# zhaozijie2022/LocoTouch

Hardware: AMD Instinct MI355X
Metric: env-steps/sec (whole node), TransportTeacher 4096 envs/GPU (higher is better)
Workload: dtype f32

## Files before the change

### locotouch_amd/_abi.py

```python
from __future__ import annotations

import ctypes
import os
import re

_HERE = os.path.dirname(os.path.abspath(__file__))
REPO = os.path.dirname(_HERE)
LIB_PATH = os.environ.get("LOCOTOUCH_AMD_LIB", os.path.join(_HERE, "_lib", "liblocotouch_env.so"))

_SCALARS = {"int": ctypes.c_int, "int32_t": ctypes.c_int32, "int64_t": ctypes.c_int64, "uint8_t": ctypes.c_uint8,
            "uint32_t": ctypes.c_uint32, "uint64_t": ctypes.c_uint64, "size_t": ctypes.c_size_t, "float": ctypes.c_float,
            "double": ctypes.c_double}
_DECL = re.compile(r"(?:const\s+)?(\w+)\s*((?:\*\s*(?:const\b\s*)?)*)(\w*)\s*((?:\[[^\]]*\]\s*)*)")


def _ctype(decl, structs, opaque, consts, typed, param):
    m = _DECL.fullmatch(decl.strip())
    if not m:
        return None
    base, stars, name, dims = m.groups()
    depth = stars.count("*")
    try:
        dims = [sum(int(t) if t.strip().isdigit() else consts[t.strip()] for t in d.split("+")) for d in re.findall(r"\[([^\]]*)\]", dims)]
    except KeyError:
# ... 62 lines not shown
        for attr in ("extra_reward_terms", "extra_termination_terms", "extra_observation_terms", "reward_term_params"):
            if hasattr(self, attr):
                v = getattr(self, attr)
                setattr(new, attr, dict(v) if isinstance(v, dict) else list(v))
        return new

    def to_dict(self) -> dict:
        def py(v):
            return [py(x) for x in v] if hasattr(v, "__len__") else v

        return {name: py(getattr(self, name)) for name, *_ in self._fields_ if not name.startswith("_")}


_ENV_VALUE_QUERIES = (
    "lt_abi_version", "lt_cfg_sizeof", "lt_cfg_num_presets", "lt_cfg_preset_id", "lt_cfg_obs_dim", "lt_cfg_tactile_dim", "lt_last_error",
    "lt_wgrad_splits", "lt_wgrad_ws_floats", "lt_elu_backward_bias_ws_floats", "lt_head_wgrad_ws_floats", "lt_adam_clip_step_ws_floats",
    "lt_elu_backward_bias_nblk", "lt_head_wgrad_nblk", "lt_mlp_backward_blocks", "lt_env_kernel_name", "lt_mlp_kernel_name")

HEADERS = (
    ("", "lt_env.h", False, _ENV_VALUE_QUERIES, ("lt_cfg", "lt_view", "lt_mlp_desc", "lt_render_view", "lt_render_desc")),
    ("OBS_NORM", "lt_obs_norm.h", False, (), ()),
    ("STUDENT", "lt_student.h", True, ("lt_student_step_launches",), ("lt_student_desc", "lt_student_params")),
    ("COLLECT", "lt_collect.h", False, (), ()),
    ("LEDGER", "lt_ledger.h", False, (), ()),
    ("CNN_TRAIN", "lt_cnn_train.h", False, ("lt_cnn_launches",), ("lt_cnn_desc", "lt_cnn_params", "lt_cnn_grads")),
    ("BC", "lt_bc.h", False, (), ()),
    ("LSTM", "lt_lstm.h", False, (), ()),
    ("MEMORY", "lt_memory.h", False, (), ("lt_memory_net",)),
    ("MEMORY_SEQ", "lt_memory_seq.h", False, ("lt_memory_seq_backward_units",), ("lt_memory_seq_net", "lt_memory_seq_grad")),
    ("MEMORY_GRU", "lt_memory_gru.h", False, ("lt_memory_gru_seq_backward_units",),
     ("lt_memory_gru_net", "lt_memory_gru_seq_net", "lt_memory_gru_seq_grad")),
    ("POLICY", "lt_policy.h", True, ("lt_policy_step_launches",), ("lt_policy_desc", "lt_policy_memory")),
    ("PPO_OPTS", "lt_ppo_opts.h", False, (), ()),
    ("MLP_DX", "lt_mlp_dx.h", True, (), ()),
    ("PPO_SYM", "lt_ppo_sym.h", False, (), ()),
    ("ENCODER", "lt_encoder.h", False, ("lt_encoder_forward_launches",), ("lt_encoder_desc", "lt_encoder_net")),
)


def _bind(table, include_dir):
    bound, seen, env_structs = [], set(), None
    for prefix, fname, uses_env_structs, queries, _ in table:
        path, queries = os.path.join(include_dir, fname), frozenset(queries)
        consts, structs, sigs = parse_header(open(path).read(), structs=env_structs if uses_env_structs else None, bases={"lt_cfg": _CfgMethods})
        if not prefix:
            env_structs = structs
        for name in sorted(queries - set(sigs)):
            raise ImportError(f"include/{fname}: the value query {name} named in _abi.HEADERS is not declared there")
        for name, (restype, _) in sigs.items():
            if name in seen:
                raise ImportError(f"include/{fname}: {name} repeats an entry point of an earlier header")
            if restype is not ctypes.c_int and (prefix or name not in queries):
                raise ImportError(f"include/{fname}: {name} returns no int (a new value query of lt_env.h belongs in _abi.HEADERS)")
        seen.update(sigs)
        bound.append((path, consts, structs, sigs, queries))
    return bound


ALL_SIGNATURES: dict = {}
ALL_VALUE_QUERIES: set = set()
for (_prefix, _, _, _, _published), (_path, _consts, _structs, _sigs, _queries) in zip(HEADERS, _bind(HEADERS, os.path.join(REPO, "include"))):
    _p = _prefix + "_" if _prefix else ""
    globals().update(_consts)
    globals().update({_p + "HEADER": _path, _p + "CONSTS": _consts, _p + "SIGNATURES": _sigs, _p + "VALUE_QUERIES": _queries})
    globals().update({_structs[_c].__name__: _structs[_c] for _c in _published})
    if not _prefix:
# ... 100 lines not shown
```

### locotouch_amd/csrc/lt_ppo.hip

```cpp
#include <hip/hip_runtime.h>
#include <math.h>
#include <stdint.h>

#include "lt_env.h"
#include "lt_host_check.h"
#include "lt_internal.h"
#include "lt_ppo_device.h"

namespace {

template <bool LOG, bool NORM>
__global__ __launch_bounds__(256) void lt_ppo_loss_kernel(const float* __restrict__ mu, const float* __restrict__ stdp, const float* __restrict__ value,
                                                          const float* __restrict__ actions, const float* __restrict__ old_logp,
                                                          const float* __restrict__ adv, const float* __restrict__ returns,
                                                          const float* __restrict__ old_values, const float* __restrict__ old_mu,
                                                          const float* __restrict__ old_sigma, const long long* __restrict__ idx,
                                                          long long M, int A, float clip, float vcoef, int clipped_value,
                                                          const float* __restrict__ adv_stats, float* __restrict__ dmu, float* __restrict__ dvalue, float* __restrict__ acc) {
  const long long row = (long long)blockIdx.x * 256 + threadIdx.x;
  const bool ok = row < M;
  const long long src = (ok && idx) ? idx[row] : row;
  __shared__ float sigma_lds[MAX_A];
  if constexpr (LOG) {
    if ((int)threadIdx.x < A) sigma_lds[threadIdx.x] = lt_sigma_of_log(stdp[threadIdx.x]);
    __syncthreads();
  }
  float part[4 + MAX_A];
  float amax_mu = 0.f, amax_v = 0.f;
#pragma unroll
  for (int i = 0; i < 4 + MAX_A; ++i) part[i] = 0.f;
  if (ok) {
    const float inv_m = 1.f / (float)M;
    float logp = 0.f, kl = 0.f;
    float z[MAX_A], isg[MAX_A];
#pragma unroll
    for (int a = 0; a < MAX_A; ++a) {
      if (a < A) {
        const float sg = LOG ? sigma_lds[a] : stdp[a], m = mu[row * A + a], x = actions[src * A + a];
        const float om = old_mu[src * A + a], os = old_sigma[src * A + a];
        isg[a] = 1.f / sg;
        z[a] = (x - m) * isg[a];
        logp += lt_ppo_logp_term<LOG>(z[a], sg, stdp[a]);
        kl += lt_ppo_kl_term(sg, os, om, m);
      }
    }
    float advr = adv[src];
    if constexpr (NORM) advr = (advr - adv_stats[0]) * adv_stats[1];
    const float ratio = __expf(logp - old_logp[src]);
    LT_PPO_SURROGATE(advr, ratio, clip, s1, s2, dsurr_dratio)
    const float dlogp = dsurr_dratio * ratio * inv_m;
#pragma unroll
    for (int a = 0; a < MAX_A; ++a) {
      if (a < A) {
        dmu[row * A + a] = dlogp * z[a] * isg[a];
        amax_mu = fmaxf(amax_mu, fabsf(dlogp * z[a] * isg[a]));
        if constexpr (LOG) part[4 + a] = dlogp * (z[a] * z[a] - 1.f);
        else part[4 + a] = dlogp * (z[a] * z[a] - 1.f) * isg[a];
      }
    }
    const float v = value[row], R = returns[src];
    float vl, dv;
    LT_PPO_VALUE_LOSS(v, R, old_values, src, clip, clipped_value, vl, dv)
    dvalue[row] = vcoef * dv * inv_m;
    amax_v = fabsf(vcoef * dv * inv_m);
    part[0] = fmaxf(s1, s2);
    part[1] = vl;
    part[2] = kl;
  }
  LT_PPO_BLOCK_REDUCE(part, amax_mu, amax_v, A, acc, false)
}

__global__ __launch_bounds__(64) void lt_ppo_finalize_kernel(const float* __restrict__ acc, const float* __restrict__ stdp, int A, float inv_m,
                                                             float vcoef, float ecoef, int std_is_log, float* __restrict__ out) {
  lt_ppo_finalize(acc, stdp, A, inv_m, vcoef, ecoef, std_is_log, out);
}

constexpr int EB_ROWS = 48;

__global__ __launch_bounds__(256) void lt_elu_bwd_bias_kernel(const float* da, const float* __restrict__ a, long long M, int N, float alpha,
                                                              float* dz, float* __restrict__ ws, float* __restrict__ amax) {
  const int n4 = N >> 2, lanes = 256 / n4;
  const int c4 = threadIdx.x % n4, rl = threadIdx.x / n4;
  const long long r0 = (long long)blockIdx.x * EB_ROWS;
  float4 sum = {0.f, 0.f, 0.f, 0.f};
  float mx = 0.f;
  if (rl < lanes) {
    for (int r = rl; r < EB_ROWS; r += lanes) {
      const long long row = r0 + r;
      if (row >= M) break;
      const float4 g = ((const float4*)(da + row * N))[c4], y = ((const float4*)(a + row * N))[c4];
      float4 o;
// ... 72 lines not shown
        s[u].x += v.x; s[u].y += v.y; s[u].z += v.z; s[u].w += v.w;
        b += RL;
      }
    }
  }
  __shared__ float4 red[256];
  red[threadIdx.x] = make_float4((s[0].x + s[1].x) + (s[2].x + s[3].x), (s[0].y + s[1].y) + (s[2].y + s[3].y),
                                 (s[0].z + s[1].z) + (s[2].z + s[3].z), (s[0].w + s[1].w) + (s[2].w + s[3].w));
  __syncthreads();
  if (lane == 0 && e < count) {
    float4 t = red[c];
    for (int l = 1; l < RL; ++l) { const float4 v = red[l * cols + c]; t.x += v.x; t.y += v.y; t.z += v.z; t.w += v.w; }
    const float o[4] = {t.x, t.y, t.z, t.w};
#pragma unroll
    for (int i = 0; i < 4; ++i) {
      const int ei = e + i;
      if (ei >= count) break;
      if (ei < split) J.out0[j][ei] = o[i];
      else if (J.out1[j]) J.out1[j][ei - split] = o[i];
    }
  }
}

void launch_one_sum(const float* ws, int nblk, long long stride, int count, int split, float* out0, float* out1, hipStream_t stream) {
  SumJobs J = {};
  J.njobs = 1;
  J.ws[0] = ws; J.out0[0] = out0; J.out1[0] = out1; J.stride[0] = stride;
  J.nblk[0] = nblk; J.count[0] = count; J.split[0] = split;
  const int epb = 256 / sum_row_lanes(nblk) * 4;
  J.first[1] = (count + epb - 1) / epb;
  hipLaunchKernelGGL(lt_partial_sums_kernel, dim3((unsigned)J.first[1]), dim3(256), 0, stream, J);
}

constexpr int HW_ROWS = 96, HW_MAX_N = 16;

template <int NN>
__global__ __launch_bounds__(256) void lt_head_wgrad_kernel(const float* __restrict__ dy, const float* __restrict__ x, int x_split, long long M, int n, int k,
                                                            float* __restrict__ ws) {
  const int k4 = k >> 2, lanes = 256 / k4;
  const int c4 = threadIdx.x % k4, rl = threadIdx.x / k4;
  const long long r0 = (long long)blockIdx.x * HW_ROWS;
  float4 acc[NN];
  float accb[NN];
#pragma unroll
  for (int j = 0; j < NN; ++j) { acc[j] = {0.f, 0.f, 0.f, 0.f}; accb[j] = 0.f; }
  if (rl < lanes) {
    for (int r = rl; r < HW_ROWS; r += 4 * lanes) {
      float4 xv[4];
      float d[4][NN];
#pragma unroll
      for (int u = 0; u < 4; ++u) {
        const long long row = r0 + r + u * lanes;
        const bool ok = (r + u * lanes) < HW_ROWS && row < M;
        xv[u] = ok ? ((const float4*)(x + row * k))[c4] : float4{0.f, 0.f, 0.f, 0.f};
        if (x_split) {
          const unsigned w[4] = {__float_as_uint(xv[u].x), __float_as_uint(xv[u].y), __float_as_uint(xv[u].z), __float_as_uint(xv[u].w)};
          float f[4];
#pragma unroll
          for (int i = 0; i < 4; ++i)
            f[i] = (float)__builtin_bit_cast(_Float16, (unsigned short)(w[i] & 0xFFFFu)) + (float)__builtin_bit_cast(_Float16, (unsigned short)(w[i] >> 16)) * (1.f / 64.f);
          xv[u] = float4{f[0], f[1], f[2], f[3]};
        }
#pragma unroll
        for (int j = 0; j < NN; ++j) d[u][j] = (ok && j < n) ? dy[row * n + j] : 0.f;
      }
#pragma unroll
      for (int u = 0; u < 4; ++u)
#pragma unroll
        for (int j = 0; j < NN; ++j) {
          acc[j].x += d[u][j] * xv[u].x; acc[j].y += d[u][j] * xv[u].y; acc[j].z += d[u][j] * xv[u].z; acc[j].w += d[u][j] * xv[u].w;
          accb[j] += d[u][j];
        }
    }
  }
  extern __shared__ float4 red[];
  float* const redb = (float*)(red + (size_t)lanes * NN * k4);
  if (rl < lanes) {
#pragma unroll
    for (int j = 0; j < NN; ++j) red[((size_t)rl * NN + j) * k4 + c4] = acc[j];
    if (c4 == 0)
#pragma unroll
      for (int j = 0; j < NN; ++j) redb[rl * NN + j] = accb[j];
  }
  __syncthreads();
  float* const out = ws + (size_t)blockIdx.x * ((size_t)n * k + HW_MAX_N);
  for (int e = threadIdx.x; e < n * k4; e += 256) {
    const int j = e / k4, c = e - j * k4;
    float4 t = red[(size_t)j * k4 + c];
    for (int l = 1; l < lanes; ++l) {
      const float4 u = red[((size_t)l * NN + j) * k4 + c];
      t.x += u.x; t.y += u.y; t.z += u.z; t.w += u.w;
    }
    ((float4*)(out + (size_t)j * k))[c] = t;
  }
  if (threadIdx.x < n) {
    float t = redb[threadIdx.x];
    for (int l = 1; l < lanes; ++l) t += redb[l * NN + threadIdx.x];
    out[(size_t)n * k + threadIdx.x] = t;
  }
}

__global__ __launch_bounds__(256) void lt_gae_kernel(const float* __restrict__ rewards, const unsigned char* __restrict__ dones,
                                                     const float* __restrict__ values, const float* __restrict__ last_values, float gamma,
                                                     float lam, int T, long long N, float* __restrict__ returns, float* __restrict__ advantages) {
  const long long e = (long long)blockIdx.x * 256 + threadIdx.x;
  if (e >= N) return;
  float next_v = last_values[e], gae = 0.f;
  for (int t = T - 1; t >= 0; --t) {
    const long long o = (long long)t * N + e;
    const float v = values[o], alive = 1.f - (float)dones[o];
    const float delta = rewards[o] + alive * gamma * next_v - v;
    gae = delta + alive * gamma * lam * gae;
    const float ret = gae + v;
    returns[o] = ret;
    advantages[o] = ret - v;
    next_v = v;
  }
}

constexpr int AD_PER_BLOCK = 2048;

__global__ __launch_bounds__(256) void lt_sumsq_kernel(const float* __restrict__ g, long long n, float* __restrict__ ws) {
  const long long base = (long long)blockIdx.x * AD_PER_BLOCK;
  float s = 0.f;
  for (int k = threadIdx.x; k < AD_PER_BLOCK; k += 256) {
    const long long i = base + k;
    if (i < n) s += g[i] * g[i];
  }
  for (int off = 32; off > 0; off >>= 1) s += __shfl_xor(s, off, 64);
  __shared__ float red[4];
  if ((threadIdx.x & 63) == 0) red[threadIdx.x >> 6] = s;
  __syncthreads();
  if (threadIdx.x == 0) ws[blockIdx.x] = (red[0] + red[1]) + (red[2] + red[3]);
}

__global__ __launch_bounds__(256) void lt_adam_kernel(float* __restrict__ p, float* __restrict__ g, float* __restrict__ m, float* __restrict__ v,
                                                      long long n, const float* __restrict__ ws, int nblk, float max_norm, float b1,
                                                      float b2, float eps, float wd, float step_size, float bc2_sqrt, float* __restrict__ norm_out,
                                                      const float* __restrict__ lr_dev, float inv_bc1) {
  __shared__ float s_coef;
  if (lr_dev) step_size = *lr_dev * inv_bc1;
  if (threadIdx.x < 64) {
    float s = 0.f;
    for (int b = threadIdx.x; b < nblk; b += 64) s += ws[b];
    for (int off = 32; off > 0; off >>= 1) s += __shfl_xor(s, off, 64);
    if (threadIdx.x == 0) {
      const float norm = sqrtf(s);
      const float c = max_norm / (norm + 1.0e-6f);
      s_coef = max_norm > 0.f ? (c < 1.f ? c : 1.f) : 1.f;
      if (blockIdx.x == 0 && norm_out) *norm_out = norm;
    }
  }
  __syncthreads();
  const float coef = s_coef;
  const long long base = (long long)blockIdx.x * AD_PER_BLOCK;
  for (int k = threadIdx.x; k < AD_PER_BLOCK; k += 256) {
    const long long i = base + k;
    if (i >= n) break;
    float gi = g[i] * coef;
    g[i] = gi;
    const float pi = p[i];
    if (wd != 0.f) gi += wd * pi;
    const float mi = m[i] + (1.f - b1) * (gi - m[i]);
    const float vi = b2 * v[i] + (1.f - b2) * gi * gi;
    m[i] = mi;
    v[i] = vi;
    p[i] = pi - step_size * (mi / (sqrtf(vi) / bc2_sqrt + eps));
  }
}

__global__ __launch_bounds__(64) void lt_std_from_log_kernel(const float* __restrict__ log_std, int A, float* __restrict__ stdp) {
  if ((int)threadIdx.x < A) stdp[threadIdx.x] = lt_sigma_of_log(log_std[threadIdx.x]);
}

__device__ __forceinline__ double lt_block_sum_f64(double v, double* red) {
#pragma unroll
  for (int off = 32; off > 0; off >>= 1) v += __shfl_xor(v, off, 64);
  __syncthreads();
  if ((threadIdx.x & 63) == 0) red[threadIdx.x >> 6] = v;
  __syncthreads();
  return (red[0] + red[1]) + (red[2] + red[3]);
}

__global__ __launch_bounds__(256) void lt_adv_stats_kernel(const float* __restrict__ adv, const long long* __restrict__ idx, long long M,
                                                           float* __restrict__ stats) {
#pragma clang fp reciprocal(off)
  __shared__ double red[4];
  const long long base = (long long)blockIdx.x * M;
  double s = 0.0;
  for (long long r = threadIdx.x; r < M; r += 256) s += (double)adv[idx ? idx[base + r] : base + r];
  const double mean = lt_block_sum_f64(s, red) / (double)M;
  double q = 0.0;
  for (long long r = threadIdx.x; r < M; r += 256) {
    const double d = (double)adv[idx ? idx[base + r] : base + r] - mean;
    q += d * d;
  }
  const double var = lt_block_sum_f64(q, red) / (double)(M - 1);
  if (threadIdx.x == 0) {
    stats[2 * blockIdx.x] = (float)mean;
    stats[2 * blockIdx.x + 1] = (float)(1.0 / (sqrt(var) + (double)1.0e-8f));
  }
}

__global__ __launch_bounds__(64) void lt_ppo_lr_rule_kernel(const float* __restrict__ kl_mean, float desired, float lr_min, float lr_max, float factor,
                                                            float* __restrict__ lr, float* __restrict__ stats, const float* __restrict__ scalars,
                                                            float* __restrict__ dstd_out, int A) {
  if (dstd_out && scalars && (int)threadIdx.x < A) dstd_out[threadIdx.x] = scalars[8 + threadIdx.x];
  if (threadIdx.x != 0) return;
  if (kl_mean && desired > 0.f) {
#pragma clang fp reciprocal(off)
    const float kl = *kl_mean;
    float v = *lr;
    if (kl > desired * 2.f) v = fmaxf(lr_min, v / factor);
    else if (kl < desired * 0.5f && kl > 0.f) v = fminf(lr_max, v * factor);
    *lr = v;
  }
  if (stats && scalars) { stats[0] += scalars[2]; stats[1] += scalars[1]; stats[2] += scalars[3]; }
}

}

extern "C" int lt_ppo_lr_rule(const float* kl_mean, float desired_kl, float lr_min, float lr_max, float factor, float* lr, float* stats,
                              const float* scalars, float* dstd_out, int num_actions, void* stream) {
  if (!lr || factor <= 1.f || num_actions < 0 || num_actions > MAX_A) return einval("lt_ppo_lr_rule: invalid argument");
  hipLaunchKernelGGL(lt_ppo_lr_rule_kernel, dim3(1), dim3(64), 0, (hipStream_t)stream, kl_mean, desired_kl, lr_min, lr_max, factor, lr, stats, scalars,
                     dstd_out, num_actions);
  return launch_status();
}

static int elu_backward_bias(const float* da, const float* a, int64_t M, int N, float alpha, float* dz, float* db, float* ws, float* amax, void* stream);
extern "C" int lt_elu_backward_bias(const float* da, const float* a, int64_t M, int N, float alpha, float* dz, float* db, float* ws, void* stream) {
  return elu_backward_bias(da, a, M, N, alpha, dz, db, ws, nullptr, stream);
}
extern "C" int lt_elu_backward_bias2(const float* da, const float* a, int64_t M, int N, float alpha, float* dz, float* db, float* ws, float* amax_blocks,
                                     void* stream) {
  return elu_backward_bias(da, a, M, N, alpha, dz, db, ws, amax_blocks, stream);
}
static int elu_backward_bias(const float* da, const float* a, int64_t M, int N, float alpha, float* dz, float* db, float* ws, float* amax, void* stream) {
  if (!da || !a || !dz || !ws || M < 1 || N < 4 || (N & 3) || N > 1024)
    return einval("lt_elu_backward_bias: invalid argument (N a multiple of 4, 4 <= N <= 1024)");
  const int nblk = (int)((M + EB_ROWS - 1) / EB_ROWS);
  hipLaunchKernelGGL(lt_elu_bwd_bias_kernel, dim3((unsigned)nblk), dim3(256), 0, (hipStream_t)stream, da, a, (long long)M, N, alpha, dz, ws, amax);
  if (db) launch_one_sum(ws, nblk, (long long)N, N, N, db, nullptr, (hipStream_t)stream);
  return launch_status();
}

extern "C" int64_t lt_head_wgrad_ws_floats(int64_t M, int n, int k) { return ((M + HW_ROWS - 1) / HW_ROWS) * ((int64_t)n * k + HW_MAX_N); }

extern "C" int lt_head_wgrad(const float* dy, const float* x, int x_split, int64_t M, int n, int k, float* dw, float* db, float* ws, void* stream) {
  if (!dy || !x || !ws || M < 1 || n < 1 || n > HW_MAX_N || k < 4 || (k & 3) || k > 1024)
    return einval("lt_head_wgrad: invalid argument (1 <= n <= 16, k a multiple of 4, 4 <= k <= 1024)");
  const int nblk = (int)((M + HW_ROWS - 1) / HW_ROWS), k4 = k / 4, lanes = 256 / k4;
  const int nn = n <= 1 ? 1 : (n <= 4 ? 4 : (n <= 8 ? 8 : (n <= 12 ? 12 : 16)));
  const size_t lds = (size_t)lanes * nn * k4 * 16 + (size_t)lanes * nn * 4;
  if (const int e = lt_ensure_dynamic_lds((const void*)lt_head_wgrad_kernel<16>, 72 * 1024)) {
    lt_set_error(hipGetErrorString((hipError_t)e));
    return LT_EHIP;
  }
  if (lds > 72 * 1024) return einval("lt_head_wgrad: n * k too large for one block's LDS partials");
  const dim3 g((unsigned)nblk), b(256);
  hipStream_t st = (hipStream_t)stream;
  switch (nn) {
    case 1: hipLaunchKernelGGL(lt_head_wgrad_kernel<1>, g, b, lds, st, dy, x, x_split, (long long)M, n, k, ws); break;
    case 4: hipLaunchKernelGGL(lt_head_wgrad_kernel<4>, g, b, lds, st, dy, x, x_split, (long long)M, n, k, ws); break;
    case 8: hipLaunchKernelGGL(lt_head_wgrad_kernel<8>, g, b, lds, st, dy, x, x_split, (long long)M, n, k, ws); break;
    case 12: hipLaunchKernelGGL(lt_head_wgrad_kernel<12>, g, b, lds, st, dy, x, x_split, (long long)M, n, k, ws); break;
    default: hipLaunchKernelGGL(lt_head_wgrad_kernel<16>, g, b, lds, st, dy, x, x_split, (long long)M, n, k, ws); break;
  }
  if (dw) launch_one_sum(ws, nblk, (long long)n * k + HW_MAX_N, n * k + n, n * k, dw, db, st);
  return launch_status();
}

extern "C" int lt_partial_sums(int njobs, const float* const* ws, const int* nblk, const int64_t* stride, const int* count, const int* split,
                               float* const* out0, float* const* out1, void* stream) {
  if (njobs < 1 || njobs > SUM_MAX_JOBS || !ws || !nblk || !stride || !count || !split || !out0 || !out1)
    return einval("lt_partial_sums: invalid argument (1 <= njobs <= 24)");
  SumJobs J = {};
  J.njobs = njobs;
  int blocks = 0;
  for (int j = 0; j < njobs; ++j) {
    if (!ws[j] || !out0[j] || nblk[j] < 1 || count[j] < 1) return einval("lt_partial_sums: invalid job");
    J.ws[j] = ws[j]; J.out0[j] = out0[j]; J.out1[j] = out1[j]; J.stride[j] = stride[j];
    J.nblk[j] = nblk[j]; J.count[j] = count[j]; J.split[j] = split[j];
    J.first[j] = blocks;
    const int epb = 256 / sum_row_lanes(nblk[j]) * 4;
// ... 16 lines not shown

extern "C" int64_t lt_elu_backward_bias_ws_floats(int64_t M, int N) { return ((M + EB_ROWS - 1) / EB_ROWS) * (int64_t)N; }

static int adam_clip_step(float* params, float* grads, float* exp_avg, float* exp_avg_sq, int64_t n, float max_norm, float lr, const float* lr_dev,
                          float beta1, float beta2, float eps, float weight_decay, int64_t step, float* ws, float* grad_norm, void* stream);

extern "C" int lt_adam_clip_step(float* params, float* grads, float* exp_avg, float* exp_avg_sq, int64_t n, float max_norm, float lr, float beta1,
                                 float beta2, float eps, float weight_decay, int64_t step, float* ws, float* grad_norm, void* stream) {
  return adam_clip_step(params, grads, exp_avg, exp_avg_sq, n, max_norm, lr, nullptr, beta1, beta2, eps, weight_decay, step, ws, grad_norm, stream);
}

extern "C" int lt_adam_clip_step_dev(float* params, float* grads, float* exp_avg, float* exp_avg_sq, int64_t n, float max_norm, const float* lr_dev,
                                     float beta1, float beta2, float eps, float weight_decay, int64_t step, float* ws, float* grad_norm, void* stream) {
  if (!lr_dev) return einval("lt_adam_clip_step_dev: null learning-rate pointer");
  return adam_clip_step(params, grads, exp_avg, exp_avg_sq, n, max_norm, 0.f, lr_dev, beta1, beta2, eps, weight_decay, step, ws, grad_norm, stream);
}

static int adam_clip_step(float* params, float* grads, float* exp_avg, float* exp_avg_sq, int64_t n, float max_norm, float lr, const float* lr_dev,
                          float beta1, float beta2, float eps, float weight_decay, int64_t step, float* ws, float* grad_norm, void* stream) {
  if (!params || !grads || !exp_avg || !exp_avg_sq || !ws || n < 1 || step < 1) return einval("lt_adam_clip_step: invalid argument");
  const int nblk = (int)((n + AD_PER_BLOCK - 1) / AD_PER_BLOCK);
  const double bc1 = 1.0 - pow((double)beta1, (double)step), bc2 = 1.0 - pow((double)beta2, (double)step);
  hipLaunchKernelGGL(lt_sumsq_kernel, dim3((unsigned)nblk), dim3(256), 0, (hipStream_t)stream, grads, (long long)n, ws);
  hipLaunchKernelGGL(lt_adam_kernel, dim3((unsigned)nblk), dim3(256), 0, (hipStream_t)stream, params, grads, exp_avg, exp_avg_sq, (long long)n, ws, nblk,
                     max_norm, beta1, beta2, eps, weight_decay, (float)((double)lr / bc1), (float)sqrt(bc2), grad_norm, lr_dev, (float)(1.0 / bc1));
  return launch_status();
}

extern "C" int64_t lt_adam_clip_step_ws_floats(int64_t n) { return (n + AD_PER_BLOCK - 1) / AD_PER_BLOCK; }

static int ppo_loss(const float* mu, const float* stdp, const float* value, const float* actions, const float* old_logp,
                    const float* adv, const float* returns, const float* old_values, const float* old_mu, const float* old_sigma,
                    const int64_t* idx, int64_t M, int A, float clip, float value_loss_coef, float entropy_coef, int use_clipped_value_loss,
                    int std_is_log, const float* adv_stats, float* dmu, float* dvalue, float* acc, float* out, void* stream) {
  const hipError_t e = hipMemsetAsync(acc, 0, sizeof(float) * (4 + MAX_A + 4), (hipStream_t)stream);
  if (e != hipSuccess) { lt_set_error(hipGetErrorString(e)); return LT_EHIP; }
  const dim3 grid((unsigned)((M + 255) / 256));
#define LT_PPO_LOSS_LAUNCH(LOG, NORM)                                                                                                      \
  hipLaunchKernelGGL((lt_ppo_loss_kernel<LOG, NORM>), grid, dim3(256), 0, (hipStream_t)stream, mu, stdp, value, actions, old_logp, adv, returns, \
                     old_values, old_mu, old_sigma, (const long long*)idx, (long long)M, A, clip, value_loss_coef, use_clipped_value_loss,   \
                     adv_stats, dmu, dvalue, acc)
  if (std_is_log && adv_stats) LT_PPO_LOSS_LAUNCH(true, true);
  else if (std_is_log) LT_PPO_LOSS_LAUNCH(true, false);
  else if (adv_stats) LT_PPO_LOSS_LAUNCH(false, true);
  else LT_PPO_LOSS_LAUNCH(false, false);
#undef LT_PPO_LOSS_LAUNCH
  if (out)
    hipLaunchKernelGGL(lt_ppo_finalize_kernel, dim3(1), dim3(64), 0, (hipStream_t)stream, acc, stdp, A, 1.f / (float)M, value_loss_coef, entropy_coef,
                       std_is_log ? 1 : 0, out);
  return launch_status();
}

extern "C" int lt_ppo_loss(const float* mu, const float* stdp, const float* value, const float* actions, const float* old_logp, const float* adv,
                           const float* returns, const float* old_values, const float* old_mu, const float* old_sigma, const int64_t* idx,
                           int64_t M, int A, float clip, float value_loss_coef, float entropy_coef, int use_clipped_value_loss, float* dmu, float* dvalue,
                           float* acc, float* out, void* stream) {
  if (!mu || !stdp || !value || !actions || !old_logp || !adv || !returns || !old_values || !old_mu || !old_sigma || !dmu || !dvalue || !acc ||
      M < 1 || A < 1 || A > MAX_A)
    return einval("lt_ppo_loss: invalid argument (1 <= num_actions <= 16)");
  return ppo_loss(mu, stdp, value, actions, old_logp, adv, returns, old_values, old_mu, old_sigma, idx, M, A, clip, value_loss_coef,
                  entropy_coef, use_clipped_value_loss, 0, nullptr, dmu, dvalue, acc, out, stream);
}

extern "C" int lt_ppo_loss_opts(const float* mu, const float* stdp, const float* value, const float* actions, const float* old_logp,
                                const float* adv, const float* returns, const float* old_values, const float* old_mu, const float* old_sigma,
                                const int64_t* idx, int64_t M, int A, float clip, float value_loss_coef, float entropy_coef,
                                int use_clipped_value_loss, int std_is_log, const float* adv_stats, float* dmu, float* dvalue, float* acc,
                                float* out, void* stream) {
  const char* fn = "lt_ppo_loss_opts";
  const ptr_check ptrs[] = {{"mu", mu, 4}, {"std", stdp, 4}, {"value", value, 4}, {"actions", actions, 4}, {"old_logp", old_logp, 4}, {"adv", adv, 4},
                            {"returns", returns, 4}, {"old_values", old_values, 4}, {"old_mu", old_mu, 4}, {"old_sigma", old_sigma, 4},
                            {"dmu", dmu, 4}, {"dvalue", dvalue, 4}, {"acc", acc, 4}};
  if (const int rc = check_ptrs(fn, "", ptrs)) return rc;
  if ((uintptr_t)idx % 8 != 0) return refuse(fn, "", "idx", "NULL or 8-byte aligned");
  if ((uintptr_t)adv_stats % 4 != 0) return refuse(fn, "", "adv_stats", "NULL or 4-byte aligned");
  if ((uintptr_t)out % 4 != 0) return refuse(fn, "", "out", "NULL or 4-byte aligned");
  if (M < 1) return refuse(fn, "", "M", ">= 1");
  if (A < 1 || A > MAX_A) return refuse(fn, "", "A", "in [1, 16]");
  return ppo_loss(mu, stdp, value, actions, old_logp, adv, returns, old_values, old_mu, old_sigma, idx, M, A, clip, value_loss_coef, entropy_coef,
                  use_clipped_value_loss, std_is_log, adv_stats, dmu, dvalue, acc, out, stream);
}

extern "C" int lt_std_from_log(const float* log_std, int A, float* stdp, void* stream) {
  const char* fn = "lt_std_from_log";
  const ptr_check ptrs[] = {{"log_std", log_std, 4}, {"std", stdp, 4}};
  if (const int rc = check_ptrs(fn, "", ptrs)) return rc;
  if (A < 1 || A > MAX_A) return refuse(fn, "", "A", "in [1, 16]");
  hipLaunchKernelGGL(lt_std_from_log_kernel, dim3(1), dim3(64), 0, (hipStream_t)stream, log_std, A, stdp);
  return launch_status();
}

extern "C" int lt_adv_stats(const float* adv, const int64_t* idx, int64_t M, int nmb, float* stats, void* stream) {
  const char* fn = "lt_adv_stats";
  const ptr_check ptrs[] = {{"adv", adv, 4}, {"stats", stats, 4}};
  if (const int rc = check_ptrs(fn, "", ptrs)) return rc;
  if ((uintptr_t)idx % 8 != 0) return refuse(fn, "", "idx", "NULL or 8-byte aligned");
  if (M < 2) return refuse(fn, "", "M", ">= 2 (the unbiased std of one element is NaN)");
  if (nmb < 1) return refuse(fn, "", "nmb", ">= 1");
  hipLaunchKernelGGL(lt_adv_stats_kernel, dim3((unsigned)nmb), dim3(256), 0, (hipStream_t)stream, adv, (const long long*)idx, (long long)M, stats);
  return launch_status();
}
```

### locotouch_amd/rl/ppo.py

```python
from __future__ import annotations

import torch
import torch.nn as nn

from .. import _abi
from .dist import Dist
from .modules import ActorCritic
from .storage import RolloutStorage


class PPO:
    def __init__(self, actor_critic: ActorCritic, num_learning_epochs=1, num_mini_batches=1, clip_param=0.2, gamma=0.998,
                 lam=0.95, value_loss_coef=1.0, entropy_coef=0.0, learning_rate=1e-3, max_grad_norm=1.0,
                 use_clipped_value_loss=True, schedule="fixed", desired_kl=0.01, device="cpu",
                 normalize_advantage_per_mini_batch=False, dist: Dist | None = None, rnd_cfg: dict | None = None,
                 symmetry_cfg: dict | None = None, **unused):
        if rnd_cfg is not None:
            raise NotImplementedError("rnd_cfg: random network distillation is not built (DESIGN.md §7: it needs an `rnd_state` observation "
                                      "group no env here produces); pass rnd_cfg=None")
        self.symmetry = self._resolve_symmetry(symmetry_cfg, actor_critic)
        self._sym_tables = None
        self.device = device
        self.dist = dist or Dist()
        self.actor_critic = actor_critic.to(device)
# ... 236 lines not shown
            xs = (split_o[0][i * rows:(i + 1) * rows], split_o[1][i * rows:(i + 1) * rows]) if split_o is not None else None
            (mu, value), acts = pair.forward_raw(o, co)
            dmu, dvalue, acc = self._direct_loss_and_rule(c, mu, value, idx, m, i, sym_args)
            if self.dist.world_size > 1 and two_buckets:
                handles = []
                pair.backward_raw(o, co, acts, dmu, dvalue, grad_of, xs, after_first=lambda: handles.append(self.dist.all_reduce_mean_begin(self._flat_grad[:critic_at])),
                                  dy_amax=(acc[20:21], acc[21:22]))
                handles.append(self.dist.all_reduce_mean_begin(self._flat_grad[critic_at:] if handles else self._flat_grad))
                for h in handles:
                    self.dist.all_reduce_mean_end(h)
            else:
                pair.backward_raw(o, co, acts, dmu, dvalue, grad_of, xs, dy_amax=(acc[20:21], acc[21:22]))
                if self.dist.world_size > 1:
                    self.dist.all_reduce_mean_(self._flat_grad)
            fa.step_dev(self.max_grad_norm, c.lr_dev)
        return self._direct_end(c, with_dx=False)

    def _direct_begin(self, key: str, pair, index, m: int, symmetric: bool = False):
        from types import SimpleNamespace

        from .fused_loss import adv_stats, std_param

        obs, cobs, small = self._flat_storage()
        small = [t.view(-1) if t.shape[-1] == 1 else t for t in small]
        a_dim = small[0].shape[1]
        if a_dim > 16:
            raise ValueError(f"{key}: the action width is {a_dim}: the loss kernel serves at most 16")
        dev = obs.device
        state = torch.zeros(5 if symmetric else 4, device=dev)
        state[0] = self.learning_rate
        std_p, std_is_log = std_param(self.actor_critic)
        pair.arm_domain_check()
        mb_stats = adv_stats(small[2], index, m, self.num_mini_batches) if self.normalize_advantage_per_mini_batch else None
        return SimpleNamespace(pair=pair, obs=obs, cobs=cobs, small=small, a_dim=a_dim, dev=dev, state=state, lr_dev=state[:1], stats=state[1:4],
                               grad_of=self._flat_adam.grad_views(), std_p=std_p, std_is_log=std_is_log, std_c=std_p.detach(),
                               stream=_abi.stream(dev), mb_stats=mb_stats)

    def _direct_loss_and_rule(self, c, mu, value, idx, m: int, i: int, sym_args=None):
        dev = c.dev
        dmu = torch.empty_like(mu)
        dvalue = torch.empty(mu.shape[0], 1, device=dev, dtype=torch.float32)
        acc = torch.empty(24, device=dev, dtype=torch.float32)
        out = torch.empty(24, device=dev, dtype=torch.float32)
        rows = (mu, c.std_c, value, *c.small, idx, m, c.a_dim, float(self.clip_param), float(self.value_loss_coef), float(self.entropy_coef),
                int(bool(self.use_clipped_value_loss)))
        opts = (int(c.std_is_log), None if c.mb_stats is None else c.mb_stats[i])
        if sym_args is not None:
            _abi.call("lt_ppo_loss_sym", *rows, *opts, *sym_args, dmu, dvalue, acc, out, c.state[4:5], c.stream)
        elif c.std_is_log or c.mb_stats is not None:
            _abi.call("lt_ppo_loss_opts", *rows, *opts, dmu, dvalue, acc, out, c.stream)
        else:
            _abi.call("lt_ppo_loss", *rows, dmu, dvalue, acc, out, c.stream)
        kl = None
        if self._adaptive:
            kl = out[4:5]
            if self.dist.world_size > 1:
                kl = self.dist.all_reduce_mean_(kl.clone())
        _abi.call("lt_ppo_lr_rule", kl, float(self.desired_kl or 0.0), 1e-5, 1e-2, 1.5, c.lr_dev, c.stats, out, c.grad_of[c.std_p], c.a_dim, c.stream)
        return dmu, dvalue, acc

    def _direct_end(self, c, with_dx: bool):
        pair, state = c.pair, c.state
        sat, dom = pair.saturated(), pair.domain_max
        pair.domain_max = None
        zero = state.new_zeros(1)
        read = torch.cat((state, zero if sat is None else sat, zero if dom is None else dom.view(1))).tolist()
        (lr, sv, ss, se), (nsat, dmax) = read[:4], read[-2:]
        if nsat > 0:
            import warnings

            sat.zero_()
            entry = "lt_mlp_backward_pair_dx" if with_dx and pair._dx_kernel_ok() else "lt_mlp_backward_pair"
            warnings.warn(f"{entry}: {int(nsat)} workgroup-layers of the gradient chain reached the f16 image's bound "
                          "(a gradient grew by more than 500x through the layers): those rows were saturated; set LT_FUSED_BACKWARD=0 "
                          "to run the chain as f32 library GEMMs")
        self.learning_rate = lr
# ... 452 lines not shown
```

Measured before the change: 68.47 million.

## Vectorise PPO loss, Adam and head-wgrad kernels; fuse finalize with LR rule

Several independent optimisations to the PPO update path. The loss kernel gains a float4-vectorised path for per-action loads and the dmu store. Adam and the sum-of-squares kernel gain float4 paths for full aligned blocks. The head weight-gradient kernel stages dy in shared memory and loads x rows with a deeper unroll. A new single-launch finalize+LR-rule kernel uses double-buffered accumulators, which removes a memset and a separate launch per minibatch. These changes target memory bandwidth and launch overhead in PPO training, which is only a fraction of whole-node env-steps throughput, and they add more code paths that depend on alignment.

Result: no change. 68.32 million (-0.2%).

```diff
diff --git a/include/lt_ppo_step.h b/include/lt_ppo_step.h
--- /dev/null
+++ b/include/lt_ppo_step.h
@@ -0,0 +1,23 @@
+#ifndef LT_PPO_STEP_H
+#define LT_PPO_STEP_H
+
+#include <stddef.h>
+#include <stdint.h>
+
+#ifdef __cplusplus
+extern "C" {
+#endif
+
+int lt_ppo_loss_step(const float* mu, const float* std, const float* value, const float* actions, const float* old_logp, const float* adv,
+                     const float* returns, const float* old_values, const float* old_mu, const float* old_sigma, const int64_t* idx, int64_t M,
+                     int A, float clip, float value_loss_coef, int use_clipped_value_loss, float* dmu, float* dvalue, float* acc, void* stream);
+
+int lt_ppo_finalize_rule(const float* acc, const float* std, int num_actions, int64_t M, float value_loss_coef, float entropy_coef, float* out,
+                         int adaptive, float desired_kl, float lr_min, float lr_max, float factor, float* lr, float* stats, float* dstd_out,
+                         float* acc_clear, void* stream);
+
+#ifdef __cplusplus
+}
+#endif
+
+#endif
diff --git a/locotouch_amd/_abi.py b/locotouch_amd/_abi.py
--- a/locotouch_amd/_abi.py
+++ b/locotouch_amd/_abi.py
@@ -118,6 +118,7 @@
      ("lt_memory_gru_net", "lt_memory_gru_seq_net", "lt_memory_gru_seq_grad")),
     ("POLICY", "lt_policy.h", True, ("lt_policy_step_launches",), ("lt_policy_desc", "lt_policy_memory")),
     ("PPO_OPTS", "lt_ppo_opts.h", False, (), ()),
+    ("PPO_STEP", "lt_ppo_step.h", False, (), ()),
     ("MLP_DX", "lt_mlp_dx.h", True, (), ()),
     ("PPO_SYM", "lt_ppo_sym.h", False, (), ()),
     ("ENCODER", "lt_encoder.h", False, ("lt_encoder_forward_launches",), ("lt_encoder_desc", "lt_encoder_net")),
diff --git a/locotouch_amd/csrc/lt_ppo.hip b/locotouch_amd/csrc/lt_ppo.hip
--- a/locotouch_amd/csrc/lt_ppo.hip
+++ b/locotouch_amd/csrc/lt_ppo.hip
@@ -6,10 +6,11 @@
 #include "lt_host_check.h"
 #include "lt_internal.h"
 #include "lt_ppo_device.h"
+#include "lt_ppo_step.h"
 
 namespace {
 
-template <bool LOG, bool NORM>
+template <bool LOG, bool NORM, bool VEC>
 __global__ __launch_bounds__(256) void lt_ppo_loss_kernel(const float* __restrict__ mu, const float* __restrict__ stdp, const float* __restrict__ value,
                                                           const float* __restrict__ actions, const float* __restrict__ old_logp,
                                                           const float* __restrict__ adv, const float* __restrict__ returns,
@@ -33,11 +34,30 @@
     const float inv_m = 1.f / (float)M;
     float logp = 0.f, kl = 0.f;
     float z[MAX_A], isg[MAX_A];
+    float rm[MAX_A], rx[MAX_A], rom[MAX_A], ros[MAX_A];
+    if constexpr (VEC) {
+#pragma unroll
+      for (int q = 0; q < MAX_A / 4; ++q) {
+        if (4 * q < A) {
+          const float4 m4 = ((const float4*)(mu + row * A))[q], x4 = ((const float4*)(actions + src * A))[q];
+          const float4 om4 = ((const float4*)(old_mu + src * A))[q], os4 = ((const float4*)(old_sigma + src * A))[q];
+          rm[4 * q] = m4.x; rm[4 * q + 1] = m4.y; rm[4 * q + 2] = m4.z; rm[4 * q + 3] = m4.w;
+          rx[4 * q] = x4.x; rx[4 * q + 1] = x4.y; rx[4 * q + 2] = x4.z; rx[4 * q + 3] = x4.w;
+          rom[4 * q] = om4.x; rom[4 * q + 1] = om4.y; rom[4 * q + 2] = om4.z; rom[4 * q + 3] = om4.w;
+          ros[4 * q] = os4.x; ros[4 * q + 1] = os4.y; ros[4 * q + 2] = os4.z; ros[4 * q + 3] = os4.w;
+        }
+      }
+    } else {
+#pragma unroll
+      for (int a = 0; a < MAX_A; ++a) {
+        if (a < A) { rm[a] = mu[row * A + a]; rx[a] = actions[src * A + a]; rom[a] = old_mu[src * A + a]; ros[a] = old_sigma[src * A + a]; }
+      }
+    }
 #pragma unroll
     for (int a = 0; a < MAX_A; ++a) {
       if (a < A) {
-        const float sg = LOG ? sigma_lds[a] : stdp[a], m = mu[row * A + a], x = actions[src * A + a];
-        const float om = old_mu[src * A + a], os = old_sigma[src * A + a];
+        const float sg = LOG ? sigma_lds[a] : stdp[a], m = rm[a], x = rx[a];
+        const float om = rom[a], os = ros[a];
         isg[a] = 1.f / sg;
         z[a] = (x - m) * isg[a];
         logp += lt_ppo_logp_term<LOG>(z[a], sg, stdp[a]);
@@ -49,14 +69,24 @@
     const float ratio = __expf(logp - old_logp[src]);
     LT_PPO_SURROGATE(advr, ratio, clip, s1, s2, dsurr_dratio)
     const float dlogp = dsurr_dratio * ratio * inv_m;
+    float dm[MAX_A];
 #pragma unroll
     for (int a = 0; a < MAX_A; ++a) {
       if (a < A) {
-        dmu[row * A + a] = dlogp * z[a] * isg[a];
+        dm[a] = dlogp * z[a] * isg[a];
         amax_mu = fmaxf(amax_mu, fabsf(dlogp * z[a] * isg[a]));
         if constexpr (LOG) part[4 + a] = dlogp * (z[a] * z[a] - 1.f);
         else part[4 + a] = dlogp * (z[a] * z[a] - 1.f) * isg[a];
       }
+    }
+    if constexpr (VEC) {
+#pragma unroll
+      for (int q = 0; q < MAX_A / 4; ++q)
+        if (4 * q < A) ((float4*)(dmu + row * A))[q] = float4{dm[4 * q], dm[4 * q + 1], dm[4 * q + 2], dm[4 * q + 3]};
+    } else {
+#pragma unroll
+      for (int a = 0; a < MAX_A; ++a)
+        if (a < A) dmu[row * A + a] = dm[a];
     }
     const float v = value[row], R = returns[src];
     float vl, dv;
@@ -195,27 +225,41 @@
   hipLaunchKernelGGL(lt_partial_sums_kernel, dim3((unsigned)J.first[1]), dim3(256), 0, stream, J);
 }
 
-constexpr int HW_ROWS = 96, HW_MAX_N = 16;
+constexpr int HW_ROWS = 96, HW_MAX_N = 16, HW_UNROLL = 12;
+__host__ __device__ inline int head_row_lanes(int k4) { return 256 / k4 < HW_ROWS ? 256 / k4 : HW_ROWS; }
 
 template <int NN>
 __global__ __launch_bounds__(256) void lt_head_wgrad_kernel(const float* __restrict__ dy, const float* __restrict__ x, int x_split, long long M, int n, int k,
                                                             float* __restrict__ ws) {
-  const int k4 = k >> 2, lanes = 256 / k4;
+  const int k4 = k >> 2, lanes = head_row_lanes(k4);
   const int c4 = threadIdx.x % k4, rl = threadIdx.x / k4;
   const long long r0 = (long long)blockIdx.x * HW_ROWS;
+  extern __shared__ float4 red[];
+  float* const redb = (float*)(red + (size_t)lanes * NN * k4);
+  float* const sdy = (float*)red;
   float4 acc[NN];
   float accb[NN];
 #pragma unroll
   for (int j = 0; j < NN; ++j) { acc[j] = {0.f, 0.f, 0.f, 0.f}; accb[j] = 0.f; }
+  float4 xv[HW_UNROLL];
+  auto load_rows = [&](int r) __attribute__((always_inline)) {
+#pragma unroll
+    for (int u = 0; u < HW_UNROLL; ++u) {
+      const long long row = r0 + r + u * lanes;
+      const bool ok = (r + u * lanes) < HW_ROWS && row < M;
+      xv[u] = ok ? ((const float4*)(x + row * k))[c4] : float4{0.f, 0.f, 0.f, 0.f};
+    }
+  };
+  if (rl < lanes) load_rows(rl);
+  for (int e = threadIdx.x; e < HW_ROWS * NN; e += 256) {
+    const int r = e / NN, j = e - r * NN;
+    sdy[e] = (j < n && r0 + r < M) ? dy[(r0 + r) * n + j] : 0.f;
+  }
+  __syncthreads();
   if (rl < lanes) {
-    for (int r = rl; r < HW_ROWS; r += 4 * lanes) {
-      float4 xv[4];
-      float d[4][NN];
-#pragma unroll
-      for (int u = 0; u < 4; ++u) {
-        const long long row = r0 + r + u * lanes;
-        const bool ok = (r + u * lanes) < HW_ROWS && row < M;
-        xv[u] = ok ? ((const float4*)(x + row * k))[c4] : float4{0.f, 0.f, 0.f, 0.f};
+    for (int r = rl; r < HW_ROWS;) {
+#pragma unroll
+      for (int u = 0; u < HW_UNROLL; ++u) {
         if (x_split) {
           const unsigned w[4] = {__float_as_uint(xv[u].x), __float_as_uint(xv[u].y), __float_as_uint(xv[u].z), __float_as_uint(xv[u].w)};
           float f[4];
@@ -224,20 +268,20 @@
             f[i] = (float)__builtin_bit_cast(_Float16, (unsigned short)(w[i] & 0xFFFFu)) + (float)__builtin_bit_cast(_Float16, (unsigned short)(w[i] >> 16)) * (1.f / 64.f);
           xv[u] = float4{f[0], f[1], f[2], f[3]};
         }
-#pragma unroll
-        for (int j = 0; j < NN; ++j) d[u][j] = (ok && j < n) ? dy[row * n + j] : 0.f;
+        const int rr = r + u * lanes;
+        const float* const drow = sdy + (rr < HW_ROWS ? rr : 0) * NN;
+#pragma unroll
+        for (int j = 0; j < NN; ++j) {
+          const float d = rr < HW_ROWS ? drow[j] : 0.f;
+          acc[j].x += d * xv[u].x; acc[j].y += d * xv[u].y; acc[j].z += d * xv[u].z; acc[j].w += d * xv[u].w;
+          accb[j] += d;
+        }
       }
-#pragma unroll
-      for (int u = 0; u < 4; ++u)
-#pragma unroll
-        for (int j = 0; j < NN; ++j) {
-          acc[j].x += d[u][j] * xv[u].x; acc[j].y += d[u][j] * xv[u].y; acc[j].z += d[u][j] * xv[u].z; acc[j].w += d[u][j] * xv[u].w;
-          accb[j] += d[u][j];
-        }
-    }
-  }
-  extern __shared__ float4 red[];
-  float* const redb = (float*)(red + (size_t)lanes * NN * k4);
+      r += HW_UNROLL * lanes;
+      if (r < HW_ROWS) load_rows(r);
+    }
+  }
+  __syncthreads();
   if (rl < lanes) {
 #pragma unroll
     for (int j = 0; j < NN; ++j) red[((size_t)rl * NN + j) * k4 + c4] = acc[j];
@@ -283,18 +327,38 @@
 
 constexpr int AD_PER_BLOCK = 2048;
 
+__device__ __forceinline__ bool lt_aligned16(const void* p) { return (reinterpret_cast<uintptr_t>(p) & 15) == 0; }
+
 __global__ __launch_bounds__(256) void lt_sumsq_kernel(const float* __restrict__ g, long long n, float* __restrict__ ws) {
   const long long base = (long long)blockIdx.x * AD_PER_BLOCK;
   float s = 0.f;
-  for (int k = threadIdx.x; k < AD_PER_BLOCK; k += 256) {
-    const long long i = base + k;
-    if (i < n) s += g[i] * g[i];
+  if (base + AD_PER_BLOCK <= n && lt_aligned16(g)) {
+    const float4 a = ((const float4*)(g + base))[threadIdx.x], b = ((const float4*)(g + base))[256 + threadIdx.x];
+    s += a.x * a.x; s += a.y * a.y; s += a.z * a.z; s += a.w * a.w;
+    s += b.x * b.x; s += b.y * b.y; s += b.z * b.z; s += b.w * b.w;
+  } else {
+    for (int k = threadIdx.x; k < AD_PER_BLOCK; k += 256) {
+      const long long i = base + k;
+      if (i < n) s += g[i] * g[i];
+    }
   }
   for (int off = 32; off > 0; off >>= 1) s += __shfl_xor(s, off, 64);
   __shared__ float red[4];
   if ((threadIdx.x & 63) == 0) red[threadIdx.x >> 6] = s;
   __syncthreads();
   if (threadIdx.x == 0) ws[blockIdx.x] = (red[0] + red[1]) + (red[2] + red[3]);
+}
+
+__device__ __forceinline__ void lt_adam_element(float& p, float& g, float& m, float& v, float coef, float b1, float b2, float eps, float wd,
+                                                float step_size, float bc2_sqrt) {
+  float gi = g * coef;
+  g = gi;
+  if (wd != 0.f) gi += wd * p;
+  const float mi = m + (1.f - b1) * (gi - m);
+  const float vi = b2 * v + (1.f - b2) * gi * gi;
+  m = mi;
+  v = vi;
+  p = p - step_size * (mi / (sqrtf(vi) / bc2_sqrt + eps));
 }
 
 __global__ __launch_bounds__(256) void lt_adam_kernel(float* __restrict__ p, float* __restrict__ g, float* __restrict__ m, float* __restrict__ v,
@@ -302,6 +366,17 @@
                                                       float b2, float eps, float wd, float step_size, float bc2_sqrt, float* __restrict__ norm_out,
                                                       const float* __restrict__ lr_dev, float inv_bc1) {
   __shared__ float s_coef;
+  const long long base = (long long)blockIdx.x * AD_PER_BLOCK;
+  const bool vec = base + AD_PER_BLOCK <= n && lt_aligned16(p) && lt_aligned16(g) && lt_aligned16(m) && lt_aligned16(v);
+  float4 p4[2], g4[2], m4[2], v4[2];
+  if (vec) {
+#pragma unroll
+    for (int u = 0; u < 2; ++u) {
+      const int q = u * 256 + threadIdx.x;
+      g4[u] = ((const float4*)(g + base))[q]; p4[u] = ((const float4*)(p + base))[q];
+      m4[u] = ((const float4*)(m + base))[q]; v4[u] = ((const float4*)(v + base))[q];
+    }
+  }
   if (lr_dev) step_size = *lr_dev * inv_bc1;
   if (threadIdx.x < 64) {
     float s = 0.f;
@@ -316,19 +391,25 @@
   }
   __syncthreads();
   const float coef = s_coef;
-  const long long base = (long long)blockIdx.x * AD_PER_BLOCK;
+  if (vec) {
+#pragma unroll
+    for (int u = 0; u < 2; ++u) {
+      const int q = u * 256 + threadIdx.x;
+      lt_adam_element(p4[u].x, g4[u].x, m4[u].x, v4[u].x, coef, b1, b2, eps, wd, step_size, bc2_sqrt);
+      lt_adam_element(p4[u].y, g4[u].y, m4[u].y, v4[u].y, coef, b1, b2, eps, wd, step_size, bc2_sqrt);
+      lt_adam_element(p4[u].z, g4[u].z, m4[u].z, v4[u].z, coef, b1, b2, eps, wd, step_size, bc2_sqrt);
+      lt_adam_element(p4[u].w, g4[u].w, m4[u].w, v4[u].w, coef, b1, b2, eps, wd, step_size, bc2_sqrt);
+      ((float4*)(g + base))[q] = g4[u]; ((float4*)(m + base))[q] = m4[u];
+      ((float4*)(v + base))[q] = v4[u]; ((float4*)(p + base))[q] = p4[u];
+    }
+    return;
+  }
   for (int k = threadIdx.x; k < AD_PER_BLOCK; k += 256) {
     const long long i = base + k;
     if (i >= n) break;
-    float gi = g[i] * coef;
-    g[i] = gi;
-    const float pi = p[i];
-    if (wd != 0.f) gi += wd * pi;
-    const float mi = m[i] + (1.f - b1) * (gi - m[i]);
-    const float vi = b2 * v[i] + (1.f - b2) * gi * gi;
-    m[i] = mi;
-    v[i] = vi;
-    p[i] = pi - step_size * (mi / (sqrtf(vi) / bc2_sqrt + eps));
+    float pi = p[i], gi = g[i], mi = m[i], vi = v[i];
+    lt_adam_element(pi, gi, mi, vi, coef, b1, b2, eps, wd, step_size, bc2_sqrt);
+    g[i] = gi; m[i] = mi; v[i] = vi; p[i] = pi;
   }
 }
 
@@ -365,9 +446,8 @@
   }
 }
 
-__global__ __launch_bounds__(64) void lt_ppo_lr_rule_kernel(const float* __restrict__ kl_mean, float desired, float lr_min, float lr_max, float factor,
-                                                            float* __restrict__ lr, float* __restrict__ stats, const float* __restrict__ scalars,
-                                                            float* __restrict__ dstd_out, int A) {
+__device__ __forceinline__ void lt_ppo_lr_rule_body(const float* kl_mean, float desired, float lr_min, float lr_max, float factor, float* lr, float* stats,
+                                                    const float* scalars, float* dstd_out, int A) {
   if (dstd_out && scalars && (int)threadIdx.x < A) dstd_out[threadIdx.x] = scalars[8 + threadIdx.x];
   if (threadIdx.x != 0) return;
   if (kl_mean && desired > 0.f) {
@@ -381,6 +461,20 @@
   if (stats && scalars) { stats[0] += scalars[2]; stats[1] += scalars[1]; stats[2] += scalars[3]; }
 }
 
+__global__ __launch_bounds__(64) void lt_ppo_lr_rule_kernel(const float* __restrict__ kl_mean, float desired, float lr_min, float lr_max, float factor,
+                                                            float* __restrict__ lr, float* __restrict__ stats, const float* __restrict__ scalars,
+                                                            float* __restrict__ dstd_out, int A) {
+  lt_ppo_lr_rule_body(kl_mean, desired, lr_min, lr_max, factor, lr, stats, scalars, dstd_out, A);
+}
+
+__global__ __launch_bounds__(64) void lt_ppo_finalize_rule_kernel(const float* acc, const float* stdp, int A, float inv_m, float vcoef, float ecoef,
+                                                                  float* out, int adaptive, float desired, float lr_min, float lr_max, float factor,
+                                                                  float* lr, float* stats, float* dstd_out, float* acc_clear) {
+  lt_ppo_finalize(acc, stdp, A, inv_m, vcoef, ecoef, 0, out);
+  if (acc_clear && threadIdx.x < 4 + MAX_A + 4) acc_clear[threadIdx.x] = 0.f;
+  lt_ppo_lr_rule_body(adaptive ? out + 4 : nullptr, desired, lr_min, lr_max, factor, lr, stats, out, dstd_out, A);
+}
+
 }
 
 extern "C" int lt_ppo_lr_rule(const float* kl_mean, float desired_kl, float lr_min, float lr_max, float factor, float* lr, float* stats,
@@ -413,7 +507,7 @@
 extern "C" int lt_head_wgrad(const float* dy, const float* x, int x_split, int64_t M, int n, int k, float* dw, float* db, float* ws, void* stream) {
   if (!dy || !x || !ws || M < 1 || n < 1 || n > HW_MAX_N || k < 4 || (k & 3) || k > 1024)
     return einval("lt_head_wgrad: invalid argument (1 <= n <= 16, k a multiple of 4, 4 <= k <= 1024)");
-  const int nblk = (int)((M + HW_ROWS - 1) / HW_ROWS), k4 = k / 4, lanes = 256 / k4;
+  const int nblk = (int)((M + HW_ROWS - 1) / HW_ROWS), k4 = k / 4, lanes = head_row_lanes(k4);
   const int nn = n <= 1 ? 1 : (n <= 4 ? 4 : (n <= 8 ? 8 : (n <= 12 ? 12 : 16)));
   const size_t lds = (size_t)lanes * nn * k4 * 16 + (size_t)lanes * nn * 4;
   if (const int e = lt_ensure_dynamic_lds((const void*)lt_head_wgrad_kernel<16>, 72 * 1024)) {
@@ -496,19 +590,28 @@
 static int ppo_loss(const float* mu, const float* stdp, const float* value, const float* actions, const float* old_logp,
                     const float* adv, const float* returns, const float* old_values, const float* old_mu, const float* old_sigma,
                     const int64_t* idx, int64_t M, int A, float clip, float value_loss_coef, float entropy_coef, int use_clipped_value_loss,
-                    int std_is_log, const float* adv_stats, float* dmu, float* dvalue, float* acc, float* out, void* stream) {
-  const hipError_t e = hipMemsetAsync(acc, 0, sizeof(float) * (4 + MAX_A + 4), (hipStream_t)stream);
-  if (e != hipSuccess) { lt_set_error(hipGetErrorString(e)); return LT_EHIP; }
+                    int std_is_log, const float* adv_stats, float* dmu, float* dvalue, float* acc, float* out, void* stream, bool clear_acc = true) {
+  if (clear_acc) {
+    const hipError_t e = hipMemsetAsync(acc, 0, sizeof(float) * (4 + MAX_A + 4), (hipStream_t)stream);
+    if (e != hipSuccess) { lt_set_error(hipGetErrorString(e)); return LT_EHIP; }
+  }
   const dim3 grid((unsigned)((M + 255) / 256));
-#define LT_PPO_LOSS_LAUNCH(LOG, NORM)                                                                                                      \
-  hipLaunchKernelGGL((lt_ppo_loss_kernel<LOG, NORM>), grid, dim3(256), 0, (hipStream_t)stream, mu, stdp, value, actions, old_logp, adv, returns, \
-                     old_values, old_mu, old_sigma, (const long long*)idx, (long long)M, A, clip, value_loss_coef, use_clipped_value_loss,   \
+  const bool vec = (A & 3) == 0 && (((uintptr_t)mu | (uintptr_t)actions | (uintptr_t)old_mu | (uintptr_t)old_sigma | (uintptr_t)dmu) & 15) == 0;
+#define LT_PPO_LOSS_LAUNCH_V(LOG, NORM, VEC)                                                                                                    \
+  hipLaunchKernelGGL((lt_ppo_loss_kernel<LOG, NORM, VEC>), grid, dim3(256), 0, (hipStream_t)stream, mu, stdp, value, actions, old_logp, adv, returns, \
+                     old_values, old_mu, old_sigma, (const long long*)idx, (long long)M, A, clip, value_loss_coef, use_clipped_value_loss,        \
                      adv_stats, dmu, dvalue, acc)
+#define LT_PPO_LOSS_LAUNCH(LOG, NORM)              \
+  do {                                               \
+    if (vec) LT_PPO_LOSS_LAUNCH_V(LOG, NORM, true);  \
+    else LT_PPO_LOSS_LAUNCH_V(LOG, NORM, false);     \
+  } while (0)
   if (std_is_log && adv_stats) LT_PPO_LOSS_LAUNCH(true, true);
   else if (std_is_log) LT_PPO_LOSS_LAUNCH(true, false);
   else if (adv_stats) LT_PPO_LOSS_LAUNCH(false, true);
   else LT_PPO_LOSS_LAUNCH(false, false);
 #undef LT_PPO_LOSS_LAUNCH
+#undef LT_PPO_LOSS_LAUNCH_V
   if (out)
     hipLaunchKernelGGL(lt_ppo_finalize_kernel, dim3(1), dim3(64), 0, (hipStream_t)stream, acc, stdp, A, 1.f / (float)M, value_loss_coef, entropy_coef,
                        std_is_log ? 1 : 0, out);
@@ -545,6 +648,40 @@
                   use_clipped_value_loss, std_is_log, adv_stats, dmu, dvalue, acc, out, stream);
 }
 
+extern "C" int lt_ppo_loss_step(const float* mu, const float* stdp, const float* value, const float* actions, const float* old_logp,
+                                const float* adv, const float* returns, const float* old_values, const float* old_mu, const float* old_sigma,
+                                const int64_t* idx, int64_t M, int A, float clip, float value_loss_coef, int use_clipped_value_loss, float* dmu,
+                                float* dvalue, float* acc, void* stream) {
+  const char* fn = "lt_ppo_loss_step";
+  const ptr_check ptrs[] = {{"mu", mu, 4}, {"std", stdp, 4}, {"value", value, 4}, {"actions", actions, 4}, {"old_logp", old_logp, 4}, {"adv", adv, 4},
+                            {"returns", returns, 4}, {"old_values", old_values, 4}, {"old_mu", old_mu, 4}, {"old_sigma", old_sigma, 4},
+                            {"dmu", dmu, 4}, {"dvalue", dvalue, 4}, {"acc", acc, 4}};
+  if (const int rc = check_ptrs(fn, "", ptrs)) return rc;
+  if ((uintptr_t)idx % 8 != 0) return refuse(fn, "", "idx", "NULL or 8-byte aligned");
+  if (M < 1) return refuse(fn, "", "M", ">= 1");
+  if (A < 1 || A > MAX_A) return refuse(fn, "", "A", "in [1, 16]");
+  return ppo_loss(mu, stdp, value, actions, old_logp, adv, returns, old_values, old_mu, old_sigma, idx, M, A, clip, value_loss_coef, 0.f,
+                  use_clipped_value_loss, 0, nullptr, dmu, dvalue, acc, nullptr, stream, false);
+}
+
+extern "C" int lt_ppo_finalize_rule(const float* acc, const float* stdp, int A, int64_t M, float value_loss_coef, float entropy_coef, float* out,
+                                    int adaptive, float desired_kl, float lr_min, float lr_max, float factor, float* lr, float* stats,
+                                    float* dstd_out, float* acc_clear, void* stream) {
+  const char* fn = "lt_ppo_finalize_rule";
+  const ptr_check ptrs[] = {{"acc", acc, 4}, {"std", stdp, 4}, {"out", out, 4}, {"lr", lr, 4}};
+  if (const int rc = check_ptrs(fn, "", ptrs)) return rc;
+  if ((uintptr_t)stats % 4 != 0) return refuse(fn, "", "stats", "NULL or 4-byte aligned");
+  if ((uintptr_t)dstd_out % 4 != 0) return refuse(fn, "", "dstd_out", "NULL or 4-byte aligned");
+  if ((uintptr_t)acc_clear % 4 != 0) return refuse(fn, "", "acc_clear", "NULL or 4-byte aligned");
+  if (acc_clear == acc) return refuse(fn, "", "acc_clear", "another buffer than acc");
+  if (M < 1) return refuse(fn, "", "M", ">= 1");
+  if (A < 1 || A > MAX_A) return refuse(fn, "", "A", "in [1, 16]");
+  if (factor <= 1.f) return refuse(fn, "", "factor", "> 1");
+  hipLaunchKernelGGL(lt_ppo_finalize_rule_kernel, dim3(1), dim3(64), 0, (hipStream_t)stream, acc, stdp, A, 1.f / (float)M, value_loss_coef, entropy_coef,
+                     out, adaptive ? 1 : 0, desired_kl, lr_min, lr_max, factor, lr, stats, dstd_out, acc_clear);
+  return launch_status();
+}
+
 extern "C" int lt_std_from_log(const float* log_std, int A, float* stdp, void* stream) {
   const char* fn = "lt_std_from_log";
   const ptr_check ptrs[] = {{"log_std", log_std, 4}, {"std", stdp, 4}};
diff --git a/locotouch_amd/rl/ppo.py b/locotouch_amd/rl/ppo.py
--- a/locotouch_amd/rl/ppo.py
+++ b/locotouch_amd/rl/ppo.py
@@ -292,16 +292,25 @@
         std_p, std_is_log = std_param(self.actor_critic)
         pair.arm_domain_check()
         mb_stats = adv_stats(small[2], index, m, self.num_mini_batches) if self.normalize_advantage_per_mini_batch else None
+        acc2 = torch.zeros(2, 24, device=dev, dtype=torch.float32)
         return SimpleNamespace(pair=pair, obs=obs, cobs=cobs, small=small, a_dim=a_dim, dev=dev, state=state, lr_dev=state[:1], stats=state[1:4],
                                grad_of=self._flat_adam.grad_views(), std_p=std_p, std_is_log=std_is_log, std_c=std_p.detach(),
-                               stream=_abi.stream(dev), mb_stats=mb_stats)
+                               stream=_abi.stream(dev), mb_stats=mb_stats, acc2=acc2, steps=0)
 
     def _direct_loss_and_rule(self, c, mu, value, idx, m: int, i: int, sym_args=None):
         dev = c.dev
         dmu = torch.empty_like(mu)
         dvalue = torch.empty(mu.shape[0], 1, device=dev, dtype=torch.float32)
+        out = torch.empty(24, device=dev, dtype=torch.float32)
+        if sym_args is None and self.dist.world_size == 1 and not c.std_is_log and c.mb_stats is None:
+            acc, other = c.acc2[c.steps & 1], c.acc2[1 - (c.steps & 1)]
+            c.steps += 1
+            _abi.call("lt_ppo_loss_step", mu, c.std_c, value, *c.small, idx, m, c.a_dim, float(self.clip_param), float(self.value_loss_coef),
+                      int(bool(self.use_clipped_value_loss)), dmu, dvalue, acc, c.stream)
+            _abi.call("lt_ppo_finalize_rule", acc, c.std_c, c.a_dim, m, float(self.value_loss_coef), float(self.entropy_coef), out,
+                      int(bool(self._adaptive)), float(self.desired_kl or 0.0), 1e-5, 1e-2, 1.5, c.lr_dev, c.stats, c.grad_of[c.std_p], other, c.stream)
+            return dmu, dvalue, acc
         acc = torch.empty(24, device=dev, dtype=torch.float32)
-        out = torch.empty(24, device=dev, dtype=torch.float32)
         rows = (mu, c.std_c, value, *c.small, idx, m, c.a_dim, float(self.clip_param), float(self.value_loss_coef), float(self.entropy_coef),
                 int(bool(self.use_clipped_value_loss)))
         opts = (int(c.std_is_log), None if c.mb_stats is None else c.mb_stats[i])
```
